# zju3dv/NeuralRecon-W

Measured on AMD Instinct MI355X. Metric: ray-samples/sec (train step) at 1024 rays x 128 samples, higher is better.
Workload: dtype f16; 1 GPU; brandenburg_gate config (BASELINE.json configs[1]): 1024 rays/GPU x (64 coarse + 64 fine) samples, SDF 8x256 + colour 4x256 + bg NeRF 8x256, 4 outside samples, up_sample_steps 2, render+loss+backward+allreduce+clip+Adam; rays_per_gpu=1024, samples_per_ray=128, global_rays=1024, parallelism=dp1, world_size=1, submission=eager, streams=2, skipped_steps=0

## Files before the change

### neuralrecon-w_amd/csrc/ncw_color.hip

```cpp
#include <stdlib.h>

#include "ncw_mlp.h"


namespace NCW_NS {

NCW_DEV void build_aux2(CVec<1>& aux, const float (&x)[3], const float (&nrm)[3], int lane) {
    const int h = lane >> 5;
#pragma unroll
    for (int r = 0; r < 16; ++r) {
        float v = 0.f;
        if (ncw_feat_of(r, 0) < 6) {
            const int f = ncw_feat_of(r, 0) + 4 * h;
            v = f == 0 ? x[0] : f == 1 ? x[1] : f == 2 ? x[2] : f == 3 ? nrm[0] : f == 4 ? nrm[1] : f == 5 ? nrm[2] : 0.f;
        }
        aux.v[0][r] = v;
    }
}

template <bool SPLIT, int RB_IN, int RB_OUT, int K_REAL, int SLOT, class P>
NCW_DEV void mma_stream_split(CVec<RB_OUT>& acc, const Act<P, RB_IN>& in, WRing& ring, const typename P::welem* __restrict__ w_hi,
                              const void* w_lo, int self_bytes, const void* w_next, int next_bytes, int lane) {
    typedef typename P::welem WE;
    if (SPLIT) {
        mma_stream<RB_IN, RB_OUT, K_REAL, SLOT>(acc, in, ring, w_hi, w_lo, self_bytes, lane);
        mma_stream<RB_IN, RB_OUT, K_REAL, SLOT>(acc, in, ring, (const WE*)w_lo, w_next, next_bytes, lane);
    } else {
        mma_stream<RB_IN, RB_OUT, K_REAL, SLOT>(acc, in, ring, w_hi, w_next, next_bytes, lane);
    }
}

template <class P, int RB>
NCW_DEV void to_act_block_hl(Act<P, RB>& hi, Act<P, RB>& lo, int rb, const f32x16& v) {
#pragma unroll
    for (int t = 0; t < 2; ++t) ncw_split8(v, t, hi.f[2 * rb + t], lo.f[2 * rb + t]);
}

template <class P, int RB>
NCW_DEV void relu_epilogue_hl(Act<P, RB>& act, Act<P, RB>& act_lo, CVec<RB>& acc, typename P::selem* st, size_t tile, int lane) {
#pragma unroll
    for (int rb = 0; rb < RB; ++rb) {
        f32x16 yv;
#pragma unroll
        for (int r = 0; r < 16; ++r) yv[r] = ncw_relu(acc.v[rb][r]);
        if (st) stash_store_block(st, tile, RB, rb, yv, lane);
        to_act_block_hl<P, RB>(act, act_lo, rb, yv);
    }
}

template <int RB_IN, int RB_OUT, int K_REAL, int SLOT, class P>
NCW_DEV void mma_stream_split3(CVec<RB_OUT>& acc, const Act<P, RB_IN>& in, const Act<P, RB_IN>& in_lo, WRing& ring,
                               const typename P::welem* __restrict__ w_hi, const void* w_lo, int self_bytes, const void* w_next,
                               int next_bytes, int lane) {
    typedef typename P::welem WE;
    mma_stream2<RB_IN, RB_OUT, K_REAL, SLOT>(acc, in, in_lo, ring, w_hi, w_lo, self_bytes, lane);
    mma_stream<RB_IN, RB_OUT, K_REAL, SLOT>(acc, in, ring, (const WE*)w_lo, w_next, next_bytes, lane);
}

template <class P, int RBF, int RBH, int RBC, bool WIDE = false>
struct ColShapes {
    static constexpr int OCC = (RBF >= 16 || WIDE) ? 1 : 2;
    static constexpr int SLOT = RingSlot<RBC, OCC>::bytes;
    static constexpr int FCB_F = ncw_first_chunk_bytes<P, RBF, 32 * RBF, RBF, SLOT>();
    static constexpr int FCB_E0 = ncw_first_chunk_bytes<P, RBF + 3, 32 * RBF + 96, RBH, SLOT>();
    static constexpr int FCB_E = ncw_first_chunk_bytes<P, RBH, 32 * RBH, RBH, SLOT>();
    static constexpr int FCB_L0 = ncw_first_chunk_bytes<P, RBH + 1, 32 * RBH + 6, RBC, SLOT>();
    static constexpr int FCB_L = ncw_first_chunk_bytes<P, RBC, 32 * RBC, RBC, SLOT>();
    static constexpr int FCB_LAST = ncw_first_chunk_bytes<P, RBC, 32 * RBC, 1, SLOT>();
    static constexpr int FCB_TLAST = ncw_first_chunk_bytes<P, 1, 3, RBC, SLOT>();
    static constexpr int FCB_TL0 = ncw_first_chunk_bytes<P, RBC, 32 * RBC, RBH + 1, SLOT>();
    static constexpr int FCB_TE0 = ncw_first_chunk_bytes<P, RBH, 32 * RBH, RBF + 3, SLOT>();
};

template <class P, int RBF, int RBH, int RBC, int SPLIT, bool TRAIN>
NCW_DEV void color_fwd_body(const NcwColorNet& net, const NcwPoints& src, int64_t n, const float* __restrict__ normals,
                            const float* __restrict__ a, const void* __restrict__ feat_stash, float* __restrict__ rgb,
                            const NcwColorStash& st) {
    typedef typename P::welem WE;
    typedef typename P::selem SE;
    auto stp = [](void* p) -> SE* { return TRAIN ? (SE*)p : nullptr; };
    typedef ColShapes<P, RBF, RBH, RBC, SPLIT == 2> SH;
    constexpr bool AS = SPLIT == 2;
    NCW_RING_DECL(SH::SLOT);
    const int lane = ncw_lane();
    ring_prologue(ring, net.w_f, SH::FCB_F);
    int64_t tile, p, ray;
    bool valid;
    tile_setup(n, tile, p, valid, lane);
    float xs[3];
    load_point(src, p, xs, ray);
    const float dir[3] = {src.rays_d[ray * 3 + 0], src.rays_d[ray * 3 + 1], src.rays_d[ray * 3 + 2]};
    const float nrm[3] = {normals[p * 3 + 0], normals[p * 3 + 1], normals[p * 3 + 2]};

    Act<P, 3> aux1a;
    {
        CVec<3> aux1;
        build_aux1<Fast<P>::v>(aux1, dir, a + ray * net.n_a, net.n_a, lane);
        if (TRAIN) stash_store<3>((SE*)st.aux1, tile, aux1, lane);
        to_act(aux1a, aux1);
        if (st.aux_bias != nullptr) ncw_act_zero3(aux1a);
    }
    Act<P, 1> aux2a, aux2lo;
    {
        CVec<1> aux2;
        build_aux2(aux2, xs, nrm, lane);
        if (TRAIN) stash_store<1>((SE*)st.aux2, tile, aux2, lane);
        if constexpr (SPLIT != 0) {
#pragma unroll
            for (int t = 0; t < 2; ++t) ncw_split8(aux2.v[0], t, aux2a.f[t], aux2lo.f[t]);
        } else {
            to_act(aux2a, aux2);
        }
    }
    Act<P, RBF + 3> cat1;
    Act<P, (AS ? RBF + 3 : 1)> cat1_lo;
    {
        Act<P, RBF> fin;
#pragma unroll
        for (int rb = 0; rb < RBF; ++rb) {
            f32x16 v;
            stash_load_block(v, (const SE*)feat_stash, tile, RBF, rb, lane);
            to_act_block<RBF>(fin, rb, v);
        }
        CVec<RBF> f;
        load_bias(f, net.b_f, lane);
        mma_stream_split<(SPLIT != 0), RBF, RBF, 32 * RBF, SH::SLOT>(f, fin, ring, (const WE*)net.w_f, net.w_f_lo, SH::FCB_F, net.w_e[0],
                                                                SH::FCB_E0, lane);
        if (TRAIN) stash_store<RBF>((SE*)st.f, tile, f, lane);
        if constexpr (AS) {
            Act<P, RBF> fa, fl;
#pragma unroll
            for (int rb = 0; rb < RBF; ++rb) to_act_block_hl<P, RBF>(fa, fl, rb, f.v[rb]);
            act_concat<RBF, 3>(cat1, fa, aux1a);
            Act<P, 3> z3;
            ncw_act_zero3(z3);
            act_concat<RBF, 3>(cat1_lo, fl, z3);
        } else {
            Act<P, RBF> fa;
            to_act(fa, f);
            act_concat<RBF, 3>(cat1, fa, aux1a);
        }
    }
    Act<P, RBH> ea;
    Act<P, (AS ? RBH : 1)> ea_lo;
    {
        CVec<RBH> e;
        load_bias(e, net.b_e[0], lane);
        if (st.aux_bias != nullptr) ncw_add_ray_bias<RBH>(e, st.aux_bias + ray * (32 * RBH), lane);
        const void* wn = net.n_head > 1 ? net.w_e[1] : net.w_l[0];
        const int nb = net.n_head > 1 ? SH::FCB_E : SH::FCB_L0;
        if constexpr (AS) {
            mma_stream_split3<RBF + 3, RBH, 32 * RBF + 96, SH::SLOT>(e, cat1, cat1_lo, ring, (const WE*)net.w_e[0], net.w_e_lo[0],
                                                                     SH::FCB_E0, wn, nb, lane);
            relu_epilogue_hl<P, RBH>(ea, ea_lo, e, stp(st.e[0]), tile, lane);
        } else {
            mma_stream_split<(SPLIT != 0), RBF + 3, RBH, 32 * RBF + 96, SH::SLOT>(e, cat1, ring, (const WE*)net.w_e[0], net.w_e_lo[0],
                                                                             SH::FCB_E0, wn, nb, lane);
            relu_epilogue<P, RBH>(ea, e, stp(st.e[0]), tile, lane);
        }
        for (int i = 1; i < net.n_head; ++i) {
            load_bias(e, net.b_e[i], lane);
            const void* wn2 = i + 1 < net.n_head ? net.w_e[i + 1] : net.w_l[0];
            const int nb2 = i + 1 < net.n_head ? SH::FCB_E : SH::FCB_L0;
            if constexpr (AS) {
                mma_stream_split3<RBH, RBH, 32 * RBH, SH::SLOT>(e, ea, ea_lo, ring, (const WE*)net.w_e[i], net.w_e_lo[i], SH::FCB_E, wn2,
                                                                nb2, lane);
                relu_epilogue_hl<P, RBH>(ea, ea_lo, e, stp(st.e[i]), tile, lane);
            } else {
                mma_stream_split<(SPLIT != 0), RBH, RBH, 32 * RBH, SH::SLOT>(e, ea, ring, (const WE*)net.w_e[i], net.w_e_lo[i], SH::FCB_E,
                                                                        wn2, nb2, lane);
                relu_epilogue<P, RBH>(ea, e, stp(st.e[i]), tile, lane);
            }
        }
    }
    Act<P, RBC> xa;
    Act<P, (AS ? RBC : 1)> xa_lo;
    CVec<RBC> x;
    const int last = net.n_lin - 1;
    {
        Act<P, RBH + 1> cat2;
        act_concat<RBH, 1>(cat2, ea, aux2a);
        load_bias(x, net.b_l[0], lane);
        if constexpr (SPLIT != 0) {
            const int nxt = 1 == last ? SH::FCB_LAST : SH::FCB_L;
            if constexpr (AS) {
                Act<P, RBH + 1> cat2lo;
#pragma unroll
                for (int i = 0; i < 2 * RBH; ++i) cat2lo.f[i] = ea_lo.f[i];
                cat2lo.f[2 * RBH] = aux2lo.f[0];
                cat2lo.f[2 * RBH + 1] = aux2lo.f[1];
                mma_stream_split3<RBH + 1, RBC, 32 * RBH + 6, SH::SLOT>(x, cat2, cat2lo, ring, (const WE*)net.w_l[0], net.w_l_lo[0], SH::FCB_L0,
                                                                        net.w_l[1], nxt, lane);
            } else {
                mma_stream<RBH + 1, RBC, 32 * RBH + 6, SH::SLOT>(x, cat2, ring, (const WE*)net.w_l[0], net.w_l_lo[0], SH::FCB_L0, lane);
                mma_stream<RBH + 1, RBC, 32 * RBH + 6, SH::SLOT>(x, cat2, ring, (const WE*)net.w_l_lo[0], net.w_l[0], SH::FCB_L0, lane);
#pragma unroll
                for (int i = 0; i < 2 * RBH; ++i)
#pragma unroll
                    for (int e = 0; e < 8; ++e) cat2.f[i][e] = (ncw_h16)0.f;
                cat2.f[2 * RBH] = aux2lo.f[0];
                cat2.f[2 * RBH + 1] = aux2lo.f[1];
                mma_stream<RBH + 1, RBC, 32 * RBH + 6, SH::SLOT>(x, cat2, ring, (const WE*)net.w_l[0], net.w_l[1], nxt, lane);
            }
        } else {
            mma_stream_split<false, RBH + 1, RBC, 32 * RBH + 6, SH::SLOT>(x, cat2, ring, (const WE*)net.w_l[0], net.w_l_lo[0], SH::FCB_L0,
                                                                          net.w_l[1], 1 == last ? SH::FCB_LAST : SH::FCB_L, lane);
        }
        if constexpr (AS) relu_epilogue_hl<P, RBC>(xa, xa_lo, x, stp(st.x[0]), tile, lane);
        else relu_epilogue<P, RBC>(xa, x, stp(st.x[0]), tile, lane);
    }
    for (int l = 1; l < last; ++l) {
        load_bias(x, net.b_l[l], lane);
        if constexpr (AS) {
            mma_stream_split3<RBC, RBC, 32 * RBC, SH::SLOT>(x, xa, xa_lo, ring, (const WE*)net.w_l[l], net.w_l_lo[l], SH::FCB_L,
                                                            net.w_l[l + 1], l + 1 == last ? SH::FCB_LAST : SH::FCB_L, lane);
            relu_epilogue_hl<P, RBC>(xa, xa_lo, x, stp(st.x[l]), tile, lane);
        } else {
            mma_stream_split<(SPLIT != 0), RBC, RBC, 32 * RBC, SH::SLOT>(x, xa, ring, (const WE*)net.w_l[l], net.w_l_lo[l], SH::FCB_L,
                                                                    net.w_l[l + 1], l + 1 == last ? SH::FCB_LAST : SH::FCB_L, lane);
            relu_epilogue<P, RBC>(xa, x, stp(st.x[l]), tile, lane);
        }
    }
    CVec<1> o;
    load_bias(o, net.b_l[last], lane);
    if constexpr (AS)
        mma_stream_split3<RBC, 1, 32 * RBC, SH::SLOT>(o, xa, xa_lo, ring, (const WE*)net.w_l[last], net.w_l_lo[last], SH::FCB_LAST,
                                                      nullptr, 0, lane);
    else
        mma_stream_split<(SPLIT != 0), RBC, 1, 32 * RBC, SH::SLOT>(o, xa, ring, (const WE*)net.w_l[last], net.w_l_lo[last], SH::FCB_LAST,
                                                              nullptr, 0, lane);
    if (valid && lane < 32) {
        rgb[p * 3 + 0] = sigmoidf_<Fast<P>::v>(o.v[0][0]);
        rgb[p * 3 + 1] = sigmoidf_<Fast<P>::v>(o.v[0][1]);
        rgb[p * 3 + 2] = sigmoidf_<Fast<P>::v>(o.v[0][2]);
    }
}

template <class P, int RBF, int RBH, int RBC, int SPLIT = 0>
__global__ __launch_bounds__(64 * NCW_WG_WAVES, ((RBF >= 16 || SPLIT == 2) ? 1 : 2)) void color_fwd_kernel(NcwColorNet net, NcwPoints src, int64_t n,
                                                                      const float* __restrict__ normals,
                                                                      const float* __restrict__ a,
                                                                      const void* __restrict__ feat_stash,
                                                                      float* __restrict__ rgb, NcwColorStash st) {
    color_fwd_body<P, RBF, RBH, RBC, SPLIT, true>(net, src, n, normals, a, feat_stash, rgb, st);
}
template <class P, int RBF, int RBH, int RBC, int SPLIT = 0>
__global__ __launch_bounds__(64 * NCW_WG_WAVES, ((RBF >= 16 || SPLIT == 2) ? 1 : 2)) void color_render_kernel(NcwColorNet net, NcwPoints src, int64_t n,
                                                                         const float* __restrict__ normals,
                                                                         const float* __restrict__ a,
                                                                         const void* __restrict__ feat_stash,
                                                                         float* __restrict__ rgb, NcwColorStash st) {
    color_fwd_body<P, RBF, RBH, RBC, SPLIT, false>(net, src, n, normals, a, feat_stash, rgb, st);
}

template <class P, int RBF, int RBH, int RBC>
__global__ __launch_bounds__(64 * NCW_WG_WAVES, (RBF >= 16 ? 1 : 2)) void color_bwd_kernel(NcwColorNet net, NcwPoints src, int64_t n,
                                                                      const float* __restrict__ rgb,
                                                                      const float* __restrict__ d_rgb,
                                                                      float* __restrict__ d_grad, float* __restrict__ d_a,
                                                                      float* __restrict__ d_a_rows,
                                                                      void* __restrict__ dfeat_stash, NcwColorStash st) {
    typedef typename P::welem WE;
    typedef typename P::selem SE;
    typedef ColShapes<P, RBF, RBH, RBC> SH;
    NCW_RING_DECL(SH::SLOT);
    const int lane = ncw_lane();
    const int last = net.n_lin - 1;
    ring_prologue(ring, net.wt_l[last], SH::FCB_TLAST);
    int64_t tile, p, ray;
    bool valid;
    tile_setup(n, tile, p, valid, lane);
    ray = (src.mode == 0) ? p : p / src.per_ray;
    const float vm = valid ? 1.f : 0.f;

    CVec<1> zo;
    cvec_zero(zo);
    if (lane < 32) {
#pragma unroll
        for (int c = 0; c < 3; ++c) {
            const float y = rgb[p * 3 + c];
            zo.v[0][c] = d_rgb[p * 3 + c] * y * (1.f - y) * vm;
        }
    }
    stash_store<1>((SE*)st.zo, tile, zo, lane);
    Act<P, 1> zoa;
    to_act(zoa, zo);
    CVec<RBC> u;
    cvec_zero(u);
    mma_stream<1, RBC, 3, SH::SLOT>(u, zoa, ring, (const WE*)net.wt_l[last], net.wt_l[last - 1],
                                    last - 1 == 0 ? SH::FCB_TL0 : SH::FCB_L, lane);
    Act<P, RBC> za;
    for (int l = last - 1; l >= 1; --l) {
        relu_backward<P, RBC>(za, u, (const SE*)st.x[l], (SE*)st.zx[l], tile, lane);
        cvec_zero(u);
        mma_stream<RBC, RBC, 32 * RBC, SH::SLOT>(u, za, ring, (const WE*)net.wt_l[l], net.wt_l[l - 1],
                                                  l - 1 == 0 ? SH::FCB_TL0 : SH::FCB_L, lane);
    }
    CVec<RBH> ue;
    {
        relu_backward<P, RBC>(za, u, (const SE*)st.x[0], (SE*)st.zx[0], tile, lane);
        CVec<RBH + 1> q;
        cvec_zero(q);
        const void* wn = net.n_head > 1 ? net.wt_e[net.n_head - 1] : net.wt_e[0];
        const int nb = net.n_head > 1 ? SH::FCB_E : SH::FCB_TE0;
        mma_stream<RBC, RBH + 1, 32 * RBC, SH::SLOT>(q, za, ring, (const WE*)net.wt_l[0], wn, nb, lane);
#pragma unroll
        for (int rb = 0; rb < RBH; ++rb) ue.v[rb] = q.v[rb];
        if (valid) {
            if (lane < 32) d_grad[p * 3 + 0] += q.v[RBH][3];
            else {
                d_grad[p * 3 + 1] += q.v[RBH][0];
                d_grad[p * 3 + 2] += q.v[RBH][1];
            }
        }
    }
    Act<P, RBH> zea;
    for (int i = net.n_head - 1; i >= 1; --i) {
        relu_backward<P, RBH>(zea, ue, (const SE*)st.e[i], (SE*)st.ze[i], tile, lane);
        cvec_zero(ue);
        mma_stream<RBH, RBH, 32 * RBH, SH::SLOT>(ue, zea, ring, (const WE*)net.wt_e[i], net.wt_e[i - 1],
                                                  i - 1 == 0 ? SH::FCB_TE0 : SH::FCB_E, lane);
    }
    {
        relu_backward<P, RBH>(zea, ue, (const SE*)st.e[0], (SE*)st.ze[0], tile, lane);
        CVec<RBF + 3> q;
        cvec_zero(q);
        mma_stream<RBH, RBF + 3, 32 * RBH, SH::SLOT>(q, zea, ring, (const WE*)net.wt_e[0], net.wt_f, SH::FCB_F, lane);
        CVec<3> qa;
        qa.v[0] = q.v[RBF]; qa.v[1] = q.v[RBF + 1]; qa.v[2] = q.v[RBF + 2];
        accumulate_d_a(qa, d_a, ray, net.n_a, valid, lane, d_a_rows, p);
        CVec<RBF> zf;
#pragma unroll
        for (int rb = 0; rb < RBF; ++rb) zf.v[rb] = q.v[rb];
        stash_store<RBF>((SE*)st.zf, tile, zf, lane);
        Act<P, RBF> zfa;
        to_act(zfa, zf);
        CVec<RBF> df;
        cvec_zero(df);
        mma_stream<RBF, RBF, 32 * RBF, SH::SLOT>(df, zfa, ring, (const WE*)net.wt_f, nullptr, 0, lane);
        stash_store<RBF>((SE*)dfeat_stash, tile, df, lane);
    }
}

}
using namespace NCW_NS;

static bool color_ok(const NcwColorNet* net) {
    return net && net->n_head >= 1 && net->n_head <= 4 && net->n_lin >= 2 && net->n_lin <= 8 && net->n_a >= 0 &&
           net->n_a <= 69;
}

#define NCW_COLOR_DISPATCH(KERNEL, ...)                                                                          \
    do {                                                                                                         \
        const int key = net->rbf * 10000 + net->rbh * 100 + net->rbc;                                            \
        if (prec == NCW_PREC_F32) {                                                                              \
            if (key == 20102) NCW_LAUNCH_TILES((KERNEL<PrecF32, 2, 1, 2>), n, st, __VA_ARGS__);                  \
            else if (key == 20408) NCW_LAUNCH_TILES((KERNEL<PrecF32, 2, 4, 8>), n, st, __VA_ARGS__);             \
            else if (key == 80408) NCW_LAUNCH_TILES((KERNEL<PrecF32, 8, 4, 8>), n, st, __VA_ARGS__);             \
            else if (key == 160408) NCW_LAUNCH_TILES((KERNEL<PrecF32, 16, 4, 8>), n, st, __VA_ARGS__);           \
            else return NCW_E_UNSUPPORTED;                                                                       \
        } else {                                                                                                 \
            if (key == 20102) NCW_LAUNCH_TILES((KERNEL<PrecBF16, 2, 1, 2>), n, st, __VA_ARGS__);                 \
            else if (key == 20408) NCW_LAUNCH_TILES((KERNEL<PrecBF16, 2, 4, 8>), n, st, __VA_ARGS__);            \
            else if (key == 80408) NCW_LAUNCH_TILES((KERNEL<PrecBF16, 8, 4, 8>), n, st, __VA_ARGS__);            \
            else if (key == 160408) NCW_LAUNCH_TILES((KERNEL<PrecBF16, 16, 4, 8>), n, st, __VA_ARGS__);          \
            else return NCW_E_UNSUPPORTED;                                                                       \
        }                                                                                                        \
    } while (0)

#ifndef NCW_HALF_F16
extern "C" int ncw_color_fwd_f16(const NcwColorNet*, int, const NcwPoints*, int64_t, const float*, const float*, const void*, float*,
                                 const NcwColorStash*, void*);
extern "C" int ncw_color_bwd_f16(const NcwColorNet*, int, const NcwPoints*, int64_t, const float*, const float*, float*, float*, float*,
                                 void*, const NcwColorStash*, void*);
#endif

extern "C" int NCW_FN(ncw_color_fwd)(const NcwColorNet* net, int prec, const NcwPoints* pts, int64_t n, const float* normals,
                                     const float* a, const void* feat_stash, float* rgb, const NcwColorStash* stash,
                                     void* stream) {
    NCW_FORWARD_F16(prec, ncw_color_fwd_f16(net, NCW_PREC_BF16, pts, n, normals, a, feat_stash, rgb, stash, stream));
    if (!color_ok(net) || !pts || !stash || n < 0 || (prec != NCW_PREC_F32 && prec != NCW_PREC_BF16)) return NCW_E_BADARG;
    if (pts->mode == 4) return NCW_E_UNSUPPORTED;
    if (n == 0) return 0;
    hipStream_t st = (hipStream_t)stream;
    const bool render = stash->aux1 == nullptr;
    if (net->w_f_lo != nullptr) {
        if (prec == NCW_PREC_F32) return NCW_E_BADARG;
        const int key = net->rbf * 10000 + net->rbh * 100 + net->rbc;
        for (int i = 0; i < net->n_head; ++i) if (net->w_e_lo[i] == nullptr) return NCW_E_BADARG;
        for (int l = 0; l < net->n_lin; ++l) if (net->w_l_lo[l] == nullptr) return NCW_E_BADARG;
#define NCW_COLOR_SPLIT_DISPATCH(KERNEL, S)                                                                                               \
        do {                                                                                                                                    \
            if (key == 20102) NCW_LAUNCH_TILES((KERNEL<PrecBF16, 2, 1, 2, S>), n, st, *net, *pts, n, normals, a, feat_stash, rgb, *stash);        \
            else if (key == 20408) NCW_LAUNCH_TILES((KERNEL<PrecBF16, 2, 4, 8, S>), n, st, *net, *pts, n, normals, a, feat_stash, rgb, *stash);   \
            else if (key == 80408) NCW_LAUNCH_TILES((KERNEL<PrecBF16, 8, 4, 8, S>), n, st, *net, *pts, n, normals, a, feat_stash, rgb, *stash);   \
            else if (key == 160408) NCW_LAUNCH_TILES((KERNEL<PrecBF16, 16, 4, 8, S>), n, st, *net, *pts, n, normals, a, feat_stash, rgb, *stash); \
            else return NCW_E_UNSUPPORTED;                                                                                                      \
        } while (0)
        if (net->act_split) {
#define NCW_COLOR_ASPLIT_DISPATCH(KERNEL)                                                                                                  \
        do {                                                                                                                                    \
            if (key == 80408) NCW_LAUNCH_TILES((KERNEL<PrecBF16, 8, 4, 8, 2>), n, st, *net, *pts, n, normals, a, feat_stash, rgb, *stash);        \
            else if (key == 160408) NCW_LAUNCH_TILES((KERNEL<PrecBF16, 16, 4, 8, 2>), n, st, *net, *pts, n, normals, a, feat_stash, rgb, *stash); \
            else return NCW_E_UNSUPPORTED;                                                                                                      \
        } while (0)
            if (render) NCW_COLOR_ASPLIT_DISPATCH(color_render_kernel);
            else NCW_COLOR_ASPLIT_DISPATCH(color_fwd_kernel);
            return 0;
        }
        if (render) NCW_COLOR_SPLIT_DISPATCH(color_render_kernel, 1);
        else NCW_COLOR_SPLIT_DISPATCH(color_fwd_kernel, 1);
        return 0;
    }
    if (render) NCW_COLOR_DISPATCH(color_render_kernel, *net, *pts, n, normals, a, feat_stash, rgb, *stash);
    else NCW_COLOR_DISPATCH(color_fwd_kernel, *net, *pts, n, normals, a, feat_stash, rgb, *stash);
    return 0;
}

extern "C" int NCW_FN(ncw_color_bwd)(const NcwColorNet* net, int prec, const NcwPoints* pts, int64_t n, const float* rgb,
                                     const float* d_rgb, float* d_grad, float* d_a, float* d_a_rows, void* dfeat_stash,
                                     const NcwColorStash* stash, void* stream) {
    NCW_FORWARD_F16(prec, ncw_color_bwd_f16(net, NCW_PREC_BF16, pts, n, rgb, d_rgb, d_grad, d_a, d_a_rows, dfeat_stash, stash, stream));
// ... 9 lines not shown
```

### neuralrecon-w_amd/csrc/ncw_common.h

```cpp
#pragma once
#include <hip/hip_runtime.h>
#include <stdint.h>
#include <type_traits>

#ifdef NCW_HALF_F16
typedef _Float16 ncw_h16;
#define NCW_MFMA_H __builtin_amdgcn_mfma_f32_32x32x16_f16
#define NCW_FN(name) name##_f16
#define NCW_NS ncw_h_f16
#else
typedef __bf16 ncw_h16;
#define NCW_MFMA_H __builtin_amdgcn_mfma_f32_32x32x16_bf16
#define NCW_FN(name) name
#define NCW_NS ncw_h_bf16
#endif
typedef ncw_h16 bf16x8 __attribute__((ext_vector_type(8)));
typedef ncw_h16 bf16x4 __attribute__((ext_vector_type(4)));
typedef float f32x16 __attribute__((ext_vector_type(16)));
typedef float f32x4 __attribute__((ext_vector_type(4)));

#define NCW_PREC_F32 0
#define NCW_PREC_BF16 1
#define NCW_PREC_F16 2
#ifdef NCW_HALF_F16
// ... 95 lines not shown
typedef __attribute__((address_space(3))) void ncw_lvoid;

typedef __attribute__((address_space(3))) char ncw_lchar;
struct WRing {
    ncw_lchar* base;
    int cur;
    int slot_bytes;
    NCW_DEV ncw_lchar* slot(int i) const { return base + i * slot_bytes; }
};

NCW_DEV void ring_issue(ncw_lchar* lds_slot, const void* gsrc, int bytes) {
    const int nw = blockDim.x >> 6;
    const int wave = __builtin_amdgcn_readfirstlane((int)(threadIdx.x >> 6));
    const int lane = threadIdx.x & 63;
    const int pieces = (bytes + 1023) >> 10;
    const char* g0 = reinterpret_cast<const char*>(gsrc) + lane * 16;
    for (int pc = wave; pc < pieces; pc += nw) {
        if (pc * 1024 + lane * 16 < bytes)
            __builtin_amdgcn_global_load_lds((ncw_gvoid*)(g0 + (size_t)pc * 1024), (ncw_lvoid*)(lds_slot + pc * 1024), 16,
                                             0, 0);
    }
}

template <class P> struct UnitsPerBlock { static constexpr int v = (P::id == NCW_PREC_F32) ? 16 : 2; };
template <class P>
NCW_HD constexpr int ncw_unit_bytes(int rb_stride) {
    return rb_stride * 64 * ((P::id == NCW_PREC_F32) ? 4 : 16);
}
NCW_HD constexpr int ncw_nb_used(int rb_in, int k_real) { return (k_real + 31) / 32 < rb_in ? (k_real + 31) / 32 : rb_in; }
template <class P>
NCW_HD constexpr int ncw_chunk_units(int rb_stride, int n_units, int slot_bytes) {
    int g = slot_bytes / ncw_unit_bytes<P>(rb_stride);
    if (g < 1) g = 1;
    return g < n_units ? g : n_units;
}
template <class P, int RB_IN, int K_REAL, int RB_STRIDE, int SLOT>
NCW_HD constexpr int ncw_first_chunk_bytes() {
    return ncw_chunk_units<P>(RB_STRIDE, ncw_nb_used(RB_IN, K_REAL) * UnitsPerBlock<P>::v, SLOT) *
           ncw_unit_bytes<P>(RB_STRIDE);
}

NCW_DEV void ring_prologue(WRing& ring, const void* w_first, int first_bytes) {
    ring.cur = 0;
    ring_issue(ring.slot(0), w_first, first_bytes);
}

template <int RB_IN>
NCW_DEV float unit_b(const Act<PrecF32, RB_IN>& in, int rb, int sub) { return in.v[rb][sub]; }
template <int RB_IN>
NCW_DEV bf16x8 unit_b(const Act<PrecBF16, RB_IN>& in, int rb, int sub) { return in.f[2 * rb + sub]; }

NCW_DEV f32x16 unit_mfma(float a, float b, const f32x16& c) { return __builtin_amdgcn_mfma_f32_32x32x2f32(a, b, c, 0, 0, 0); }
NCW_DEV f32x16 unit_mfma(const bf16x8& a, const bf16x8& b, const f32x16& c) {
    return NCW_MFMA_H(a, b, c, 0, 0, 0);
}

template <class P>
NCW_HD constexpr int ncw_unit_first_feature(int rb, int sub) {
    return (P::id == NCW_PREC_F32) ? 32 * rb + ncw_feat_of(sub, 0) : 16 * (2 * rb + sub);
}

template <class P, int RB_IN_>
struct ActB {
    static constexpr int RB_IN = RB_IN_;
    const Act<P, RB_IN_>& a;
    NCW_DEV explicit ActB(const Act<P, RB_IN_>& a_) : a(a_) {}
    NCW_DEV void prepare(int) {}
    NCW_DEV auto b(int rb, int sub) const { return unit_b<RB_IN_>(a, rb, sub); }
};

template <class P, int RA, int RG>
struct CatB {
    static constexpr int RB_IN = RA + RG;
    const Act<P, RA>& a;
    const Act<P, RG>& g;
    NCW_DEV CatB(const Act<P, RA>& a_, const Act<P, RG>& g_) : a(a_), g(g_) {}
    NCW_DEV void prepare(int) {}
    NCW_DEV auto b(int rb, int sub) const {
        return rb < RA ? unit_b<RA>(a, rb < RA ? rb : 0, sub) : unit_b<RG>(g, rb >= RA ? rb - RA : 0, sub);
    }
};

struct NoB2 {};
template <int RB_OUT, int K_REAL, int SLOT, int RB_STRIDE, class P, class BP, bool PIPE = (SLOT != 32768) && (RB_OUT <= 8), class BP2 = NoB2>
NCW_DEV void mma_stream_b(CVec<RB_OUT>& acc, BP& bp, WRing& ring, const typename P::welem* __restrict__ wp,
                          const void* w_next, int next_bytes, int lane, BP2* bp2 = nullptr) {
    constexpr int RB_IN = BP::RB_IN;
    constexpr int UPB = UnitsPerBlock<P>::v;
    constexpr int NU = ncw_nb_used(RB_IN, K_REAL) * UPB;
    constexpr int UB = ncw_unit_bytes<P>(RB_STRIDE);
    constexpr int CU = ncw_chunk_units<P>(RB_STRIDE, NU, SLOT);
    constexpr int NCH = (NU + CU - 1) / CU;
    typedef typename std::conditional<P::id == NCW_PREC_F32, float, bf16x8>::type Frag;
#pragma unroll
    for (int c = 0; c < NCH; ++c) {
        __syncthreads();
        if (c + 1 < NCH) {
            const int nu = (c + 2) * CU <= NU ? CU : NU - (c + 1) * CU;
            ring_issue(ring.slot(ring.cur ^ 1), reinterpret_cast<const char*>(wp) + (size_t)(c + 1) * CU * UB, nu * UB);
        } else if (w_next != nullptr) {
            ring_issue(ring.slot(ring.cur ^ 1), w_next, next_bytes);
        }
        typedef const __attribute__((address_space(3))) Frag* lfrag_t;
        lfrag_t lw = (lfrag_t)(ring.slot(ring.cur)) + lane;
        Frag cur[RB_OUT], nxt[RB_OUT];
        bool loaded = false;
#pragma unroll
        for (int u = 0; u < CU; ++u) {
            const int q = c * CU + u;
            if (q >= NU) continue;
            const int rb = q / UPB, sub = q % UPB;
            if (sub == 0) bp.prepare(rb);
            if (ncw_unit_first_feature<P>(rb, sub) >= K_REAL) continue;
            if (!loaded) {
#pragma unroll
                for (int ro = 0; ro < RB_OUT; ++ro) cur[ro] = (lw + u * RB_STRIDE * 64)[ro * 64];
                loaded = true;
            }
            int un = -1;
#pragma unroll
            for (int v = CU - 1; v > u; --v) {
                const int qv = c * CU + v;
                if (qv < NU && ncw_unit_first_feature<P>(qv / UPB, qv % UPB) < K_REAL) un = v;
            }
            if (PIPE && un >= 0) {
#pragma unroll
                for (int ro = 0; ro < RB_OUT; ++ro) nxt[ro] = (lw + un * RB_STRIDE * 64)[ro * 64];
                __builtin_amdgcn_sched_barrier(0);
            }
            const auto b = bp.b(rb, sub);
#pragma unroll
            for (int ro = 0; ro < RB_OUT; ++ro) acc.v[ro] = unit_mfma(cur[ro], b, acc.v[ro]);
            if constexpr (!std::is_same<BP2, NoB2>::value) {
                const auto b2 = bp2->b(rb, sub);
#pragma unroll
                for (int ro = 0; ro < RB_OUT; ++ro) acc.v[ro] = unit_mfma(cur[ro], b2, acc.v[ro]);
            }
            if (PIPE && un >= 0) {
                __builtin_amdgcn_sched_barrier(0);
#pragma unroll
                for (int ro = 0; ro < RB_OUT; ++ro) cur[ro] = nxt[ro];
            } else {
                loaded = false;
                if (RB_OUT > 8) __builtin_amdgcn_sched_barrier(0);
            }
        }
        ring.cur ^= 1;
    }
}

template <int RB_IN, int RB_OUT, int K_REAL, int SLOT, int RB_STRIDE = RB_OUT, class P>
NCW_DEV void mma_stream(CVec<RB_OUT>& acc, const Act<P, RB_IN>& in, WRing& ring, const typename P::welem* __restrict__ wp,
                        const void* w_next, int next_bytes, int lane) {
    ActB<P, RB_IN> bp(in);
    mma_stream_b<RB_OUT, K_REAL, SLOT, RB_STRIDE, P>(acc, bp, ring, wp, w_next, next_bytes, lane);
}
template <int RB_IN, int RB_OUT, int K_REAL, int SLOT, int RB_STRIDE = RB_OUT, class P>
NCW_DEV void mma_stream2(CVec<RB_OUT>& acc, const Act<P, RB_IN>& in, const Act<P, RB_IN>& in2, WRing& ring,
                         const typename P::welem* __restrict__ wp, const void* w_next, int next_bytes, int lane) {
    ActB<P, RB_IN> bp(in), bp2(in2);
    mma_stream_b<RB_OUT, K_REAL, SLOT, RB_STRIDE, P, ActB<P, RB_IN>, (SLOT != 32768) && (RB_OUT <= 8), ActB<P, RB_IN>>(
        acc, bp, ring, wp, w_next, next_bytes, lane, &bp2);
}

template <int A, int B>
NCW_DEV void act_concat(Act<PrecF32, A + B>& o, const Act<PrecF32, A>& x, const Act<PrecF32, B>& y) {
#pragma unroll
    for (int i = 0; i < A; ++i) o.v[i] = x.v[i];
#pragma unroll
    for (int i = 0; i < B; ++i) o.v[A + i] = y.v[i];
}
template <int A, int B>
NCW_DEV void act_concat(Act<PrecBF16, A + B>& o, const Act<PrecBF16, A>& x, const Act<PrecBF16, B>& y) {
#pragma unroll
    for (int i = 0; i < 2 * A; ++i) o.f[i] = x.f[i];
#pragma unroll
    for (int i = 0; i < 2 * B; ++i) o.f[2 * A + i] = y.f[i];
}

NCW_HD constexpr size_t ncw_packed_elems(int rb_out, int rb_in) { return (size_t)rb_out * rb_in * 1024; }

template <int RB>
NCW_DEV void load_bias(CVec<RB>& acc, const float* __restrict__ bp, int lane) {
    const int h = lane >> 5;
#pragma unroll
    for (int rb = 0; rb < RB; ++rb) {
        const f32x4* b4 = reinterpret_cast<const f32x4*>(bp + (rb * 2 + h) * 16);
// ... 256 lines not shown
```

### neuralrecon-w_amd/csrc/ncw_mlp.h

```cpp
#pragma once
#include "../../include/neuconw_hip.h"
#include "ncw_common.h"

template <class P>
struct Fast { static constexpr bool v = (P::id == NCW_PREC_BF16); };

NCW_DEV void ncw_lds_barrier() {
    asm volatile("s_waitcnt lgkmcnt(0)" ::: "memory");
    __builtin_amdgcn_s_barrier();
    asm volatile("" ::: "memory");
}

NCW_DEV float grid_linspace(float start, float end, int steps, int i) {
    if (steps == 1) return start;
    const float step = (end - start) / (float)(steps - 1);
    return (i < steps / 2) ? start + step * (float)i : end - step * (float)(steps - 1 - i);
}

NCW_DEV int64_t points_count(const NcwPoints& s, int64_t n) {
    if (s.mode != 4) return n;
    const int64_t c = (int64_t)s.count[0];
    return c < n ? c : n;
}
NCW_DEV int64_t point_slot(const NcwPoints& s, int64_t p) { return s.mode == 4 ? (int64_t)s.idx[p] : p; }
// ... 48 lines not shown
        NCW_STASH_ST(p[g * 64], t);
    }
}
template <class SE>
NCW_DEV void stash_store_block_keep(SE* __restrict__ base, size_t tile, int RB, int rb, const f32x16& v, int lane) {
    NCW_EXP_STORE_HOOK();
    typedef SE vec4 __attribute__((ext_vector_type(4)));
    vec4* p = reinterpret_cast<vec4*>(base) + ((tile * RB + rb) * 4) * 64 + lane;
#pragma unroll
    for (int g = 0; g < 4; ++g) {
        vec4 t;
#pragma unroll
        for (int c = 0; c < 4; ++c) t[c] = (SE)v[4 * g + c];
        p[g * 64] = t;
    }
}
template <class SE>
NCW_DEV void stash_load_block(f32x16& v, const SE* __restrict__ base, size_t tile, int RB, int rb, int lane) {
    NCW_EXP_LOAD_HOOK(v);
    typedef SE vec4 __attribute__((ext_vector_type(4)));
    const vec4* p = reinterpret_cast<const vec4*>(base) + ((tile * RB + rb) * 4) * 64 + lane;
#pragma unroll
    for (int g = 0; g < 4; ++g) {
        vec4 t = NCW_STASH_LD(p[g * 64]);
#pragma unroll
        for (int c = 0; c < 4; ++c) v[4 * g + c] = (float)t[c];
    }
}
template <int RB>
NCW_DEV void to_act_block(Act<PrecF32, RB>& a, int rb, const f32x16& v) { a.v[rb] = v; }
template <int RB>
NCW_DEV void to_act_block(Act<PrecBF16, RB>& a, int rb, const f32x16& v) {
#pragma unroll
    for (int t = 0; t < 2; ++t)
#pragma unroll
        for (int e = 0; e < 8; ++e) a.f[2 * rb + t][e] = (ncw_h16)v[8 * t + e];
}

template <class P, int RB>
NCW_DEV void softplus_epilogue(Act<P, RB>& act, CVec<RB>& acc, typename P::selem* st_h, typename P::selem* st_s,
                               size_t tile, int lane) {
#pragma unroll
    for (int rb = 0; rb < RB; ++rb) {
        f32x16 yv, sv;
#pragma unroll
        for (int r = 0; r < 16; ++r) {
            float y, s;
            softplus100<Fast<P>::v>(acc.v[rb][r], y, s);
            yv[r] = y;
            sv[r] = s;
        }
        if (st_s) stash_store_block(st_s, tile, RB, rb, sv, lane);
        if (st_h) stash_store_block_keep(st_h, tile, RB, rb, yv, lane);
        to_act_block<RB>(act, rb, yv);
    }
}

template <class P, int RB>
NCW_DEV void relu_epilogue(Act<P, RB>& act, CVec<RB>& acc, typename P::selem* st, size_t tile, int lane) {
#pragma unroll
    for (int rb = 0; rb < RB; ++rb) {
        f32x16 yv;
#pragma unroll
        for (int r = 0; r < 16; ++r) yv[r] = ncw_relu(acc.v[rb][r]);
        if (st) stash_store_block(st, tile, RB, rb, yv, lane);
        to_act_block<RB>(act, rb, yv);
    }
}

template <class P, int RB>
NCW_DEV void relu_backward(Act<P, RB>& za, const CVec<RB>& u, const typename P::selem* st_y, typename P::selem* st_z,
                           size_t tile, int lane) {
#pragma unroll
    for (int rb = 0; rb < RB; ++rb) {
        f32x16 y, z;
        stash_load_block(y, st_y, tile, RB, rb, lane);
#pragma unroll
        for (int r = 0; r < 16; ++r) z[r] = y[r] > 0.f ? u.v[rb][r] : 0.f;
        stash_store_block(st_z, tile, RB, rb, z, lane);
        to_act_block<RB>(za, rb, z);
    }
}

template <class P, int RB, int NX = 0>
struct SoftplusB {
    static constexpr int RB_IN = RB + NX;
    typedef typename P::selem SE;
    const CVec<RB>& z;
    SE* st_h;
    SE* st_s;
    size_t tile;
    int lane;
    const Act<P, (NX > 0 ? NX : 1)>* extra;
    Act<P, RB> act;
    NCW_DEV SoftplusB(const CVec<RB>& z_, SE* h, SE* s, size_t t, int l, const Act<P, (NX > 0 ? NX : 1)>* x = nullptr)
        : z(z_), st_h(h), st_s(s), tile(t), lane(l), extra(x) {}
    NCW_DEV void prepare(int rb) {
        if (rb >= RB) return;
        f32x16 yv, sv;
#pragma unroll
        for (int r = 0; r < 16; ++r) {
            float y, sg;
            softplus100<Fast<P>::v>(z.v[rb][r], y, sg);
            yv[r] = y;
            sv[r] = sg;
        }
        if (st_s) stash_store_block(st_s, tile, RB, rb, sv, lane);
        if (st_h) stash_store_block_keep(st_h, tile, RB, rb, yv, lane);
        to_act_block<RB>(act, rb, yv);
    }
    NCW_DEV auto b(int rb, int sub) const {
        if constexpr (NX > 0) {
            if (rb >= RB) return unit_b<NX>(*extra, rb - RB, sub);
        }
        return unit_b<RB>(act, rb < RB ? rb : 0, sub);
    }
};

template <class P, int RB, int NX = 0>
struct ReluB {
    static constexpr int RB_IN = RB + NX;
    typedef typename P::selem SE;
    const CVec<RB>& z;
    SE* st;
    size_t tile;
    int lane;
    const Act<P, (NX > 0 ? NX : 1)>* extra;
    Act<P, RB> act;
    NCW_DEV ReluB(const CVec<RB>& z_, SE* s, size_t t, int l, const Act<P, (NX > 0 ? NX : 1)>* x = nullptr)
        : z(z_), st(s), tile(t), lane(l), extra(x) {}
    NCW_DEV void prepare(int rb) {
        if (rb >= RB) return;
        f32x16 yv;
#pragma unroll
        for (int r = 0; r < 16; ++r) yv[r] = ncw_relu(z.v[rb][r]);
        if (st) stash_store_block(st, tile, RB, rb, yv, lane);
        to_act_block<RB>(act, rb, yv);
    }
    NCW_DEV auto b(int rb, int sub) const {
        if constexpr (NX > 0) {
            if (rb >= RB) return unit_b<NX>(*extra, rb - RB, sub);
        }
        return unit_b<RB>(act, rb < RB ? rb : 0, sub);
    }
};

template <class P, int RB, int NX = 0>
struct LinearB {
    static constexpr int RB_IN = RB + NX;
    typedef typename P::selem SE;
    const CVec<RB>& z;
    SE* st;
    size_t tile;
    int lane;
    const Act<P, (NX > 0 ? NX : 1)>* extra;
    Act<P, RB> act;
    NCW_DEV LinearB(const CVec<RB>& z_, SE* s, size_t t, int l, const Act<P, (NX > 0 ? NX : 1)>* x = nullptr)
        : z(z_), st(s), tile(t), lane(l), extra(x) {}
    NCW_DEV void prepare(int rb) {
        if (rb >= RB) return;
        if (st) stash_store_block(st, tile, RB, rb, z.v[rb], lane);
        to_act_block<RB>(act, rb, z.v[rb]);
    }
    NCW_DEV auto b(int rb, int sub) const {
        if constexpr (NX > 0) {
            if (rb >= RB) return unit_b<NX>(*extra, rb - RB, sub);
        }
        return unit_b<RB>(act, rb < RB ? rb : 0, sub);
    }
};

template <int RB>
NCW_DEV void cvec_copy(CVec<RB>& d, const CVec<RB>& s) {
#pragma unroll
    for (int i = 0; i < RB; ++i) d.v[i] = s.v[i];
}

#define NCW_WG_WAVES 4
#define NCW_LAUNCH_TILES(kernel, n, st, ...)                                                         \
    do {                                                                                            \
        const int64_t tiles__ = ((n) + 31) / 32;                                                    \
        const int64_t blocks__ = (tiles__ + NCW_WG_WAVES - 1) / NCW_WG_WAVES;                       \
        hipLaunchKernelGGL(kernel, dim3((unsigned)blocks__), dim3(64 * NCW_WG_WAVES), 0, st, __VA_ARGS__); \
        NCW_CHECK_LAUNCH();                                                                         \
    } while (0)

template <int RB, int OCC = 1>
struct RingSlot { static constexpr int bytes = RB >= 8 ? (OCC >= 2 ? 32768 : 65536) : 16384; };

#define NCW_RING_DECL(SLOTB)                                              \
    __shared__ __attribute__((aligned(16))) char ring_mem__[2 * (SLOTB)]; \
    WRing ring;                                                           \
    ring.base = (ncw_lchar*)ring_mem__;                                   \
    ring.cur = 0;                                                         \
    ring.slot_bytes = (SLOTB)

template <bool FAST>
NCW_DEV void build_aux1(CVec<3>& aux, const float (&dir)[3], const float* __restrict__ a_row, int n_a, int lane) {
    const int h = lane >> 5;
#pragma unroll
    for (int rb = 0; rb < 3; ++rb)
#pragma unroll
        for (int r = 0; r < 16; ++r) {
            const int f = 32 * rb + ncw_feat_of(r, 0) + 4 * h;
            float v;
            if (32 * rb + ncw_feat_of(r, 0) + 4 < 27) {
                v = freq_feature<3, 4, FAST>(dir, f);
            } else if (32 * rb + ncw_feat_of(r, 0) >= 27) {
                v = (f - 27 < n_a) ? a_row[f - 27] : 0.f;
            } else {
                v = (f < 27) ? freq_feature<3, 4, FAST>(dir, f) : ((f - 27 < n_a) ? a_row[f - 27] : 0.f);
            }
            aux.v[rb][r] = v;
        }
}

NCW_DEV void ncw_act_zero3(Act<PrecF32, 3>& a) {
#pragma unroll
    for (int i = 0; i < 3; ++i)
#pragma unroll
        for (int r = 0; r < 16; ++r) a.v[i][r] = 0.f;
}
NCW_DEV void ncw_act_zero3(Act<PrecBF16, 3>& a) {
#pragma unroll
    for (int i = 0; i < 6; ++i)
#pragma unroll
        for (int e = 0; e < 8; ++e) a.f[i][e] = (ncw_h16)0.f;
}
NCW_DEV void ncw_add_ray_bias_block(f32x16& v, const float* __restrict__ row, int rb, int lane) {
    const f32x4* ab = reinterpret_cast<const f32x4*>(row) + 8 * rb + (lane >> 5);
#pragma unroll
    for (int g = 0; g < 4; ++g) {
        const f32x4 t = ab[2 * g];
#pragma unroll
        for (int c = 0; c < 4; ++c) v[4 * g + c] += t[c];
    }
}
template <int RB>
NCW_DEV void ncw_add_ray_bias(CVec<RB>& e, const float* __restrict__ row, int lane) {
#pragma unroll
    for (int rb = 0; rb < RB; ++rb) ncw_add_ray_bias_block(e.v[rb], row, rb, lane);
}

NCW_DEV void accumulate_d_a(const CVec<3>& q, float* __restrict__ d_a, int64_t ray, int n_a, bool valid, int lane,
                            float* __restrict__ rows = nullptr, int64_t p = 0) {
    const int h = lane >> 5;
    if (rows != nullptr) {
#pragma unroll
        for (int rb = 0; rb < 3; ++rb)
#pragma unroll
            for (int r = 0; r < 16; ++r) {
                if (32 * rb + ncw_feat_of(r, 0) + 4 < 27) continue;
                const int j = 32 * rb + ncw_feat_of(r, 0) + 4 * h - 27;
                if (valid && j >= 0 && j < n_a) rows[p * n_a + j] = q.v[rb][r];
            }
        return;
    }
    const int64_t r0 = __shfl(ray, 0, 64);
    const bool uniform = __all((ray == r0) ? 1 : 0);
#pragma unroll
    for (int rb = 0; rb < 3; ++rb)
#pragma unroll
        for (int r = 0; r < 16; ++r) {
            if (32 * rb + ncw_feat_of(r, 0) + 4 < 27) continue;
            const int f = 32 * rb + ncw_feat_of(r, 0) + 4 * h;
            const int j = f - 27;
            float v = valid ? q.v[rb][r] : 0.f;
            if (uniform) {
#pragma unroll
                for (int o = 1; o < 32; o <<= 1) v += __shfl_xor(v, o, 64);
                if ((lane & 31) == 0 && j >= 0 && j < n_a) atomicAdd(d_a + ray * n_a + j, v);
            } else {
                if (valid && j >= 0 && j < n_a) atomicAdd(d_a + ray * n_a + j, v);
            }
        }
}
```

Before: 32.82 million ray-samples/s.

## Prefetch stash blocks and weight fragments ahead in color backward kernel

The color MLP backward kernel gains a register fragment ring for 16-bit modes, so LDS weight fragments are loaded several MFMAs ahead under scheduling barriers. Stashed activations for the ReLU backward are requested one block ahead, including across layer boundaries, to hide global-load latency. The forward path hoists the appearance-embedding loads ahead of the frequency-feature maths and skips building aux1 in render mode when a ray bias is present. Unused SoftplusB, ReluB and LinearB helper structs are deleted. The main cost is added register pressure, which could lower occupancy or cause spills.

After: 32.78 million ray-samples/s. No clear change (-0.1%).

```diff
diff --git a/neuralrecon-w_amd/csrc/ncw_color.hip b/neuralrecon-w_amd/csrc/ncw_color.hip
--- a/neuralrecon-w_amd/csrc/ncw_color.hip
+++ b/neuralrecon-w_amd/csrc/ncw_color.hip
@@ -92,10 +92,14 @@
     const float dir[3] = {src.rays_d[ray * 3 + 0], src.rays_d[ray * 3 + 1], src.rays_d[ray * 3 + 2]};
     const float nrm[3] = {normals[p * 3 + 0], normals[p * 3 + 1], normals[p * 3 + 2]};
 
+    constexpr bool INFLIGHT = RBF < 16 || SPLIT == 2;
     Act<P, 3> aux1a;
-    {
+    if (INFLIGHT && !TRAIN && st.aux_bias != nullptr) {
+        ncw_act_zero3(aux1a);
+    } else {
         CVec<3> aux1;
-        build_aux1<Fast<P>::v>(aux1, dir, a + ray * net.n_a, net.n_a, lane);
+        if constexpr (INFLIGHT) build_aux1_inflight<Fast<P>::v>(aux1, dir, a + ray * net.n_a, net.n_a, lane);
+        else build_aux1<Fast<P>::v>(aux1, dir, a + ray * net.n_a, net.n_a, lane);
         if (TRAIN) stash_store<3>((SE*)st.aux1, tile, aux1, lane);
         to_act(aux1a, aux1);
         if (st.aux_bias != nullptr) ncw_act_zero3(aux1a);
@@ -253,6 +257,23 @@
     color_fwd_body<P, RBF, RBH, RBC, SPLIT, false>(net, src, n, normals, a, feat_stash, rgb, st);
 }
 
+template <int FRING, int RB_IN, int RB_OUT, int K_REAL, int SLOT, class P>
+NCW_DEV void mma_stream_r(CVec<RB_OUT>& acc, const Act<P, RB_IN>& in, WRing& ring, const typename P::welem* __restrict__ wp,
+                          const void* w_next, int next_bytes, int lane) {
+    if constexpr (FRING > 0) {
+        ActB<P, RB_IN> bp(in);
+        mma_stream_b<RB_OUT, K_REAL, SLOT, RB_OUT, P, ActB<P, RB_IN>, false, NoB2, FRING>(acc, bp, ring, wp, w_next, next_bytes, lane);
+    } else {
+        mma_stream<RB_IN, RB_OUT, K_REAL, SLOT>(acc, in, ring, wp, w_next, next_bytes, lane);
+    }
+}
+template <bool AHEAD, class P, int RB>
+NCW_DEV void relu_back(Act<P, RB>& za, const CVec<RB>& u, const StashRaw<typename P::selem>& y0, const typename P::selem* st_y,
+                       typename P::selem* st_z, size_t tile, int lane) {
+    if constexpr (AHEAD) relu_backward_ahead<P, RB>(za, u, y0, st_y, st_z, tile, lane);
+    else relu_backward<P, RB>(za, u, st_y, st_z, tile, lane);
+}
+
 template <class P, int RBF, int RBH, int RBC>
 __global__ __launch_bounds__(64 * NCW_WG_WAVES, (RBF >= 16 ? 1 : 2)) void color_bwd_kernel(NcwColorNet net, NcwPoints src, int64_t n,
                                                                       const float* __restrict__ rgb,
@@ -263,6 +284,8 @@
     typedef typename P::welem WE;
     typedef typename P::selem SE;
     typedef ColShapes<P, RBF, RBH, RBC> SH;
+    constexpr int FRING = P::id == NCW_PREC_F32 ? 0 : 4;
+    constexpr bool AHEAD = P::id != NCW_PREC_F32;
     NCW_RING_DECL(SH::SLOT);
     const int lane = ncw_lane();
     const int last = net.n_lin - 1;
@@ -287,23 +310,27 @@
     to_act(zoa, zo);
     CVec<RBC> u;
     cvec_zero(u);
-    mma_stream<1, RBC, 3, SH::SLOT>(u, zoa, ring, (const WE*)net.wt_l[last], net.wt_l[last - 1],
+    StashRaw<SE> y0;
+    if (AHEAD) stash_request_block(y0, (const SE*)st.x[last - 1], tile, RBC, 0, lane);
+    mma_stream_r<FRING, 1, RBC, 3, SH::SLOT>(u, zoa, ring, (const WE*)net.wt_l[last], net.wt_l[last - 1],
                                     last - 1 == 0 ? SH::FCB_TL0 : SH::FCB_L, lane);
     Act<P, RBC> za;
     for (int l = last - 1; l >= 1; --l) {
-        relu_backward<P, RBC>(za, u, (const SE*)st.x[l], (SE*)st.zx[l], tile, lane);
+        relu_back<AHEAD, P, RBC>(za, u, y0, (const SE*)st.x[l], (SE*)st.zx[l], tile, lane);
         cvec_zero(u);
-        mma_stream<RBC, RBC, 32 * RBC, SH::SLOT>(u, za, ring, (const WE*)net.wt_l[l], net.wt_l[l - 1],
+        if (AHEAD) stash_request_block(y0, (const SE*)st.x[l - 1], tile, RBC, 0, lane);
+        mma_stream_r<FRING, RBC, RBC, 32 * RBC, SH::SLOT>(u, za, ring, (const WE*)net.wt_l[l], net.wt_l[l - 1],
                                                   l - 1 == 0 ? SH::FCB_TL0 : SH::FCB_L, lane);
     }
     CVec<RBH> ue;
     {
-        relu_backward<P, RBC>(za, u, (const SE*)st.x[0], (SE*)st.zx[0], tile, lane);
+        relu_back<AHEAD, P, RBC>(za, u, y0, (const SE*)st.x[0], (SE*)st.zx[0], tile, lane);
         CVec<RBH + 1> q;
         cvec_zero(q);
+        if (AHEAD) stash_request_block(y0, (const SE*)st.e[net.n_head - 1], tile, RBH, 0, lane);
         const void* wn = net.n_head > 1 ? net.wt_e[net.n_head - 1] : net.wt_e[0];
         const int nb = net.n_head > 1 ? SH::FCB_E : SH::FCB_TE0;
-        mma_stream<RBC, RBH + 1, 32 * RBC, SH::SLOT>(q, za, ring, (const WE*)net.wt_l[0], wn, nb, lane);
+        mma_stream_r<FRING, RBC, RBH + 1, 32 * RBC, SH::SLOT>(q, za, ring, (const WE*)net.wt_l[0], wn, nb, lane);
 #pragma unroll
         for (int rb = 0; rb < RBH; ++rb) ue.v[rb] = q.v[rb];
         if (valid) {
@@ -316,16 +343,17 @@
     }
     Act<P, RBH> zea;
     for (int i = net.n_head - 1; i >= 1; --i) {
-        relu_backward<P, RBH>(zea, ue, (const SE*)st.e[i], (SE*)st.ze[i], tile, lane);
+        relu_back<AHEAD, P, RBH>(zea, ue, y0, (const SE*)st.e[i], (SE*)st.ze[i], tile, lane);
         cvec_zero(ue);
-        mma_stream<RBH, RBH, 32 * RBH, SH::SLOT>(ue, zea, ring, (const WE*)net.wt_e[i], net.wt_e[i - 1],
+        if (AHEAD) stash_request_block(y0, (const SE*)st.e[i - 1], tile, RBH, 0, lane);
+        mma_stream_r<FRING, RBH, RBH, 32 * RBH, SH::SLOT>(ue, zea, ring, (const WE*)net.wt_e[i], net.wt_e[i - 1],
                                                   i - 1 == 0 ? SH::FCB_TE0 : SH::FCB_E, lane);
     }
     {
-        relu_backward<P, RBH>(zea, ue, (const SE*)st.e[0], (SE*)st.ze[0], tile, lane);
+        relu_back<AHEAD, P, RBH>(zea, ue, y0, (const SE*)st.e[0], (SE*)st.ze[0], tile, lane);
         CVec<RBF + 3> q;
         cvec_zero(q);
-        mma_stream<RBH, RBF + 3, 32 * RBH, SH::SLOT>(q, zea, ring, (const WE*)net.wt_e[0], net.wt_f, SH::FCB_F, lane);
+        mma_stream_r<FRING, RBH, RBF + 3, 32 * RBH, SH::SLOT>(q, zea, ring, (const WE*)net.wt_e[0], net.wt_f, SH::FCB_F, lane);
         CVec<3> qa;
         qa.v[0] = q.v[RBF]; qa.v[1] = q.v[RBF + 1]; qa.v[2] = q.v[RBF + 2];
         accumulate_d_a(qa, d_a, ray, net.n_a, valid, lane, d_a_rows, p);
@@ -337,7 +365,7 @@
         to_act(zfa, zf);
         CVec<RBF> df;
         cvec_zero(df);
-        mma_stream<RBF, RBF, 32 * RBF, SH::SLOT>(df, zfa, ring, (const WE*)net.wt_f, nullptr, 0, lane);
+        mma_stream_r<FRING, RBF, RBF, 32 * RBF, SH::SLOT>(df, zfa, ring, (const WE*)net.wt_f, nullptr, 0, lane);
         stash_store<RBF>((SE*)dfeat_stash, tile, df, lane);
     }
 }
diff --git a/neuralrecon-w_amd/csrc/ncw_common.h b/neuralrecon-w_amd/csrc/ncw_common.h
--- a/neuralrecon-w_amd/csrc/ncw_common.h
+++ b/neuralrecon-w_amd/csrc/ncw_common.h
@@ -201,7 +201,8 @@
 };
 
 struct NoB2 {};
-template <int RB_OUT, int K_REAL, int SLOT, int RB_STRIDE, class P, class BP, bool PIPE = (SLOT != 32768) && (RB_OUT <= 8), class BP2 = NoB2>
+template <int RB_OUT, int K_REAL, int SLOT, int RB_STRIDE, class P, class BP, bool PIPE = (SLOT != 32768) && (RB_OUT <= 8), class BP2 = NoB2,
+          int RING = 0>
 NCW_DEV void mma_stream_b(CVec<RB_OUT>& acc, BP& bp, WRing& ring, const typename P::welem* __restrict__ wp,
                           const void* w_next, int next_bytes, int lane, BP2* bp2 = nullptr) {
     constexpr int RB_IN = BP::RB_IN;
@@ -222,6 +223,30 @@
         }
         typedef const __attribute__((address_space(3))) Frag* lfrag_t;
         lfrag_t lw = (lfrag_t)(ring.slot(ring.cur)) + lane;
+        if constexpr (RING > 0) {
+            static_assert(P::id != NCW_PREC_F32 && UPB == 2, "fragment ring: 16-bit modes");
+            constexpr int NAU = (K_REAL + 15) / 16 < NU ? (K_REAL + 15) / 16 : NU;
+            const int na = NAU - c * CU < CU ? (NAU - c * CU > 0 ? NAU - c * CU : 0) : CU;
+            const int nf = na * RB_OUT;
+            Frag fr[RING];
+#pragma unroll
+            for (int j = 0; j < RING; ++j)
+                if (j < nf) fr[j] = (lw + (j / RB_OUT) * RB_STRIDE * 64)[(j % RB_OUT) * 64];
+            __builtin_amdgcn_sched_barrier(0);
+#pragma unroll
+            for (int j = 0; j < CU * RB_OUT; ++j) {
+                if (j >= nf) continue;
+                const int q = c * CU + j / RB_OUT, ro = j % RB_OUT;
+                if (ro == 0 && q % UPB == 0) bp.prepare(q / UPB);
+                acc.v[ro] = unit_mfma(fr[j % RING], bp.b(q / UPB, q % UPB), acc.v[ro]);
+                if constexpr (!std::is_same<BP2, NoB2>::value)
+                    acc.v[ro] = unit_mfma(fr[j % RING], bp2->b(q / UPB, q % UPB), acc.v[ro]);
+                if (j + RING < nf) fr[j % RING] = (lw + ((j + RING) / RB_OUT) * RB_STRIDE * 64)[((j + RING) % RB_OUT) * 64];
+                __builtin_amdgcn_sched_barrier(0);
+            }
+            ring.cur ^= 1;
+            continue;
+        }
         Frag cur[RB_OUT], nxt[RB_OUT];
         bool loaded = false;
 #pragma unroll
diff --git a/neuralrecon-w_amd/csrc/ncw_mlp.h b/neuralrecon-w_amd/csrc/ncw_mlp.h
--- a/neuralrecon-w_amd/csrc/ncw_mlp.h
+++ b/neuralrecon-w_amd/csrc/ncw_mlp.h
@@ -154,93 +154,34 @@
     }
 }
 
-template <class P, int RB, int NX = 0>
-struct SoftplusB {
-    static constexpr int RB_IN = RB + NX;
-    typedef typename P::selem SE;
-    const CVec<RB>& z;
-    SE* st_h;
-    SE* st_s;
-    size_t tile;
-    int lane;
-    const Act<P, (NX > 0 ? NX : 1)>* extra;
-    Act<P, RB> act;
-    NCW_DEV SoftplusB(const CVec<RB>& z_, SE* h, SE* s, size_t t, int l, const Act<P, (NX > 0 ? NX : 1)>* x = nullptr)
-        : z(z_), st_h(h), st_s(s), tile(t), lane(l), extra(x) {}
-    NCW_DEV void prepare(int rb) {
-        if (rb >= RB) return;
-        f32x16 yv, sv;
-#pragma unroll
-        for (int r = 0; r < 16; ++r) {
-            float y, sg;
-            softplus100<Fast<P>::v>(z.v[rb][r], y, sg);
-            yv[r] = y;
-            sv[r] = sg;
-        }
-        if (st_s) stash_store_block(st_s, tile, RB, rb, sv, lane);
-        if (st_h) stash_store_block_keep(st_h, tile, RB, rb, yv, lane);
-        to_act_block<RB>(act, rb, yv);
-    }
-    NCW_DEV auto b(int rb, int sub) const {
-        if constexpr (NX > 0) {
-            if (rb >= RB) return unit_b<NX>(*extra, rb - RB, sub);
-        }
-        return unit_b<RB>(act, rb < RB ? rb : 0, sub);
-    }
+template <class SE>
+struct StashRaw {
+    typedef SE vec4 __attribute__((ext_vector_type(4)));
+    vec4 t[4];
 };
-
-template <class P, int RB, int NX = 0>
-struct ReluB {
-    static constexpr int RB_IN = RB + NX;
-    typedef typename P::selem SE;
-    const CVec<RB>& z;
-    SE* st;
-    size_t tile;
-    int lane;
-    const Act<P, (NX > 0 ? NX : 1)>* extra;
-    Act<P, RB> act;
-    NCW_DEV ReluB(const CVec<RB>& z_, SE* s, size_t t, int l, const Act<P, (NX > 0 ? NX : 1)>* x = nullptr)
-        : z(z_), st(s), tile(t), lane(l), extra(x) {}
-    NCW_DEV void prepare(int rb) {
-        if (rb >= RB) return;
-        f32x16 yv;
-#pragma unroll
-        for (int r = 0; r < 16; ++r) yv[r] = ncw_relu(z.v[rb][r]);
-        if (st) stash_store_block(st, tile, RB, rb, yv, lane);
-        to_act_block<RB>(act, rb, yv);
-    }
-    NCW_DEV auto b(int rb, int sub) const {
-        if constexpr (NX > 0) {
-            if (rb >= RB) return unit_b<NX>(*extra, rb - RB, sub);
-        }
-        return unit_b<RB>(act, rb < RB ? rb : 0, sub);
-    }
-};
-
-template <class P, int RB, int NX = 0>
-struct LinearB {
-    static constexpr int RB_IN = RB + NX;
-    typedef typename P::selem SE;
-    const CVec<RB>& z;
-    SE* st;
-    size_t tile;
-    int lane;
-    const Act<P, (NX > 0 ? NX : 1)>* extra;
-    Act<P, RB> act;
-    NCW_DEV LinearB(const CVec<RB>& z_, SE* s, size_t t, int l, const Act<P, (NX > 0 ? NX : 1)>* x = nullptr)
-        : z(z_), st(s), tile(t), lane(l), extra(x) {}
-    NCW_DEV void prepare(int rb) {
-        if (rb >= RB) return;
-        if (st) stash_store_block(st, tile, RB, rb, z.v[rb], lane);
-        to_act_block<RB>(act, rb, z.v[rb]);
-    }
-    NCW_DEV auto b(int rb, int sub) const {
-        if constexpr (NX > 0) {
-            if (rb >= RB) return unit_b<NX>(*extra, rb - RB, sub);
-        }
-        return unit_b<RB>(act, rb < RB ? rb : 0, sub);
-    }
-};
+template <class SE>
+NCW_DEV void stash_request_block(StashRaw<SE>& y, const SE* __restrict__ base, size_t tile, int RB, int rb, int lane) {
+    typedef typename StashRaw<SE>::vec4 vec4;
+    const vec4* p = reinterpret_cast<const vec4*>(base) + ((tile * RB + rb) * 4) * 64 + lane;
+#pragma unroll
+    for (int g = 0; g < 4; ++g) y.t[g] = NCW_STASH_LD(p[g * 64]);
+}
+template <class P, int RB>
+NCW_DEV void relu_backward_ahead(Act<P, RB>& za, const CVec<RB>& u, const StashRaw<typename P::selem>& y0,
+                                 const typename P::selem* st_y, typename P::selem* st_z, size_t tile, int lane) {
+    StashRaw<typename P::selem> y = y0;
+#pragma unroll
+    for (int rb = 0; rb < RB; ++rb) {
+        StashRaw<typename P::selem> yn = y;
+        if (rb + 1 < RB) stash_request_block(yn, st_y, tile, RB, rb + 1, lane);
+        f32x16 z;
+#pragma unroll
+        for (int r = 0; r < 16; ++r) z[r] = (float)y.t[r >> 2][r & 3] > 0.f ? u.v[rb][r] : 0.f;
+        stash_store_block(st_z, tile, RB, rb, z, lane);
+        to_act_block<RB>(za, rb, z);
+        y = yn;
+    }
+}
 
 template <int RB>
 NCW_DEV void cvec_copy(CVec<RB>& d, const CVec<RB>& s) {
@@ -287,6 +228,39 @@
         }
 }
 
+template <bool FAST>
+NCW_DEV void build_aux1_inflight(CVec<3>& aux, const float (&dir)[3], const float* __restrict__ a_row, int n_a, int lane) {
+    const int h = lane >> 5;
+    CVec<3> av;
+    if (n_a > 0) {
+#pragma unroll
+        for (int rb = 0; rb < 3; ++rb)
+#pragma unroll
+            for (int r = 0; r < 16; ++r) {
+                if (32 * rb + ncw_feat_of(r, 0) + 4 < 27) continue;
+                const int j = 32 * rb + ncw_feat_of(r, 0) + 4 * h - 27;
+                av.v[rb][r] = a_row[j < 0 ? 0 : (j < n_a ? j : n_a - 1)];
+            }
+    } else {
+        cvec_zero(av);
+    }
+#pragma unroll
+    for (int rb = 0; rb < 3; ++rb)
+#pragma unroll
+        for (int r = 0; r < 16; ++r) {
+            const int f = 32 * rb + ncw_feat_of(r, 0) + 4 * h;
+            float v;
+            if (32 * rb + ncw_feat_of(r, 0) + 4 < 27) {
+                v = freq_feature<3, 4, FAST>(dir, f);
+            } else if (32 * rb + ncw_feat_of(r, 0) >= 27) {
+                v = (f - 27 < n_a) ? av.v[rb][r] : 0.f;
+            } else {
+                v = (f < 27) ? freq_feature<3, 4, FAST>(dir, f) : ((f - 27 < n_a) ? av.v[rb][r] : 0.f);
+            }
+            aux.v[rb][r] = v;
+        }
+}
+
 NCW_DEV void ncw_act_zero3(Act<PrecF32, 3>& a) {
 #pragma unroll
     for (int i = 0; i < 3; ++i)
```
